# qurAI-amsterdam/SuperResolution_aniso_MRI

Hardware: AMD Instinct MI355X
Metric: training slices/sec (ae_combined, 160x160, latent=128) (higher is better)
Workload: dtype f32; 1 GPU; ACDC synthetic 12x(3x1x160x160) triplets, ae_combined latent=128 depth=32 scales=2, MSE synthesis loss (BASELINE configs[1]); global_batch_triplets=12, parallelism=dp1, init=reference Initializer, seed 892372, random weights, launch=captured HIP graph replay

## Files before the change

### superresolution_aniso_mri_amd/_hip.py

```python
import ctypes
import os
from ctypes import c_char_p, c_double, c_float, c_int, c_int64, c_size_t, c_void_p

import torch

_HERE = os.path.dirname(os.path.abspath(__file__))
LIB_PATH = os.path.join(_HERE, "libaesr_hip.so")
if os.environ.get("AESR_LIB"):
    import sys as _sys
    LIB_PATH = os.path.abspath(os.environ["AESR_LIB"])
    _sys.stderr.write("[aesr] AESR_LIB: loading the VARIANT library %s (not the shipped libaesr_hip.so)\n" % LIB_PATH)

P = c_void_p
IP = ctypes.POINTER(c_int)
FP = ctypes.POINTER(c_float)
DP = ctypes.POINTER(c_double)

class TripletDesc(ctypes.Structure):
    _fields_ = [("vol_off", ctypes.c_longlong), ("H", c_int), ("W", c_int), ("z_from", c_int), ("z_to", c_int), ("z_between", c_int),
                ("oy", c_int), ("ox", c_int), ("k", c_int), ("gain", c_float), ("cutoff", c_float)]


class WgradReduceJob(ctypes.Structure):
    _fields_ = [("workspace", c_void_p), ("dw", c_void_p), ("db", c_void_p), ("N", c_int), ("H", c_int), ("W", c_int), ("Cin", c_int),
# ... 110 lines not shown
    "aesr_conv2d_wino_fwd": (c_int, [P, P, P, P] + [c_int] * 6 + [c_float, P]),
    "aesr_conv2d_wino_dgrad": (c_int, [P, P, P, P] + [c_int] * 6 + [c_float, P]),
    "aesr_conv2d_wino_workspace_floats": (c_size_t, [c_int] * 6),
    "aesr_conv2d_wino_fwd_bn_supported": (c_int, [c_int] * 5),
    "aesr_conv2d_wino_fwd_bn": (c_int, [P, P, P, P, P, P] + [c_int] * 6 + [c_float, c_int, P]),
    "aesr_conv2d_wino_fwd_ws": (c_int, [P, P, P, P, P, c_size_t] + [c_int] * 6 + [c_float, P]),
    "aesr_conv2d_wino_dgrad_ws": (c_int, [P, P, P, P, P, c_size_t] + [c_int] * 6 + [c_float, P]),
    "aesr_conv2d_wino_fwd_up2": (c_int, [P, P, P, P] + [c_int] * 6 + [c_float, P]),
    "aesr_conv2d_wino_dgrad_sum2": (c_int, [P, P, P] + [c_int] * 5 + [P]),
    "aesr_conv2d_wgrad_up2_supported": (c_int, [c_int, c_int]),
    "aesr_conv2d_wgrad_up2": (c_int, [P, P, P, P, P] + [c_int] * 5 + [P]),
    "aesr_conv2d_wgrad_partial": (c_int, [P, P, P] + [c_int] * 8 + [P]),
    "aesr_conv2d_wgrad_reduce_many": (c_int, [ctypes.POINTER(WgradReduceJob), c_int, P]),
    "aesr_comm_rccl_version": (c_int, [IP]),
    "aesr_comm_unique_id": (c_int, [c_char_p]),
    "aesr_comm_init": (c_int, [c_char_p, c_int, c_int, ctypes.POINTER(c_void_p)]),
    "aesr_comm_destroy": (c_int, [P]),
    "aesr_comm_abort": (c_int, [P]),
    "aesr_comm_allreduce": (c_int, [P, P, c_size_t, c_int, c_int, P]),
    "aesr_comm_allreduce_many": (c_int, [P, ctypes.POINTER(c_void_p), ctypes.POINTER(c_size_t), c_int, c_int, c_int, P]),
    "aesr_comm_broadcast": (c_int, [P, P, c_size_t, c_int, c_int, P]),
}
SIGNATURES_PREPROC = {
    "aesr_inplane_out_size": (c_int, [c_int, c_double]),
    "aesr_inplane_workspace_bytes": (c_size_t, [c_int, c_int]),
    "aesr_inplane_resample": (c_int, [P, P, P] + [c_int] * 5 + [DP, c_int, DP, c_int, IP, DP, IP, DP, c_int, P]),
}
SIGNATURES_DATAPREP = {
    "aesr_thick_slices_out_slices": (c_int, [c_int, c_int]),
    "aesr_thick_slices_store_bytes": (c_int, [c_int, P, P]),
    "aesr_thick_slices": (c_int, [P, P, c_int, c_int, c_int, c_int, DP, c_int, P]),
    "aesr_triplet_assemble_raw": (c_int, [P, ctypes.POINTER(TripletDesc), c_int, c_int, P, P, P]),
}
P2P_HANDLE_BYTES, P2P_SLOTS = 64, 32
COMM_ID_BYTES = 128
COMM_F32, COMM_F64, COMM_SUM, COMM_MAX = 0, 1, 0, 1

ACT_NONE, ACT_LRELU, ACT_RELU, ACT_SIGMOID = 0, 1, 2, 3
BN_NONE, BN_POOL, BN_UP = 0, 1, 2
RS_POOL, RS_NEAREST, RS_BILINEAR = 1, 2, 3
BN_NWG = 512
REDUCE_MAX_JOBS = 16
MSE_NPART = 512
MSE3_WS = 3 * 256 + 1
LPIPS_NCH = 64


def _load():
    if not os.path.exists(LIB_PATH):
        raise RuntimeError(
            "libaesr_hip.so not found at %s -- build it with `python __graft_entry__.py` (or `make -C "
            "superresolution_aniso_mri_amd/csrc`). The HIP extension is mandatory: there is no CPU/eager fallback." % LIB_PATH)
    lib = ctypes.CDLL(LIB_PATH)
    for name, (res, args) in list(SIGNATURES.items()) + list(SIGNATURES_PREPROC.items()) + list(SIGNATURES_DATAPREP.items()):
        fn = getattr(lib, name, None)
        if fn is None:
            raise RuntimeError("libaesr_hip.so does not export %s (stale build?)" % name)
        fn.restype, fn.argtypes = res, args
    return lib


lib = _load()


def last_error():
    return lib.aesr_last_error_string().decode("utf-8", "replace")


def check(rc, what):
    if rc != 0:
        raise RuntimeError("%s failed (code %d): %s" % (what, rc, last_error()))


def check_device_watchdogs(where):
    nb = int(lib.aesr_bn_fused1_timeouts())
    if nb:
        raise RuntimeError("%s: the one-launch BatchNorm kernel's grid barrier gave up %d time(s) in this process -- its workgroups were not all "
                           "resident (the device is shared with another grid-barrier kernel: set AESR_BN_FUSED=0); results since are not "
                           "trustworthy; nothing was written" % (where, nb))
    n = int(lib.aesr_conv2d_wino_ring_timeouts())
    if n:
        raise RuntimeError("%s: the ring convolution kernel's arrival-counter watchdog fired %d time(s) in this process -- activations / "
                           "gradients computed since are not trustworthy (csrc/conv_wino_ring.hip: wait_full); nothing was written" % (where, n))


def ptr(t):
    if t is None:
# ... 35 lines not shown
```

### superresolution_aniso_mri_amd/csrc/aesr_api.hip

```cpp
#include <stdarg.h>
#include <stdio.h>
#include <stdlib.h>
#include <string.h>

#include <map>
#include <mutex>
#include <tuple>

#include "../../include/aesr_hip.h"
#include "../../include/aesr_hip_dataprep.h"
#include "aesr_kernels.h"

static thread_local char g_err[512] = "";
void aesr_set_error(const char* fmt, ...) {
    va_list ap;
    va_start(ap, fmt);
    vsnprintf(g_err, sizeof(g_err), fmt, ap);
    va_end(ap);
}

static void cout_padding(int Cout, int* CoutP, int* NB) {
    if (Cout <= 16) { *CoutP = 16; *NB = 1; }
    else if (Cout <= 32) { *CoutP = 32; *NB = 2; }
    else { *CoutP = round_up(Cout, 64); *NB = 4; }
}

static bool conv_dims_ok(int N, int H, int W, int Cin, int Cout) {
    if (N < 1 || H < 1 || W < 1 || Cin < 1 || Cout < 1) return false;
    if (N > (1 << 24) || H > (1 << 15) || W > (1 << 15) || Cin > (1 << 15) || Cout > (1 << 15)) return false;
    const unsigned long long px = (unsigned long long)N * (unsigned)(H + 2) * (unsigned)(W + 2);
    return px * (unsigned long long)(Cin > Cout ? Cin : Cout) < 0x1C000000ull;
}
#define AESR_CHECK_DIMS(who, N, H, W, Cin, Cout)                                                                                            \
    do {                                                                                                                                    \
        if (!conv_dims_ok(N, H, W, Cin, Cout)) {                                                                                            \
            aesr_set_error("%s: %d x %d x %d with %d -> %d channels is empty or beyond the kernels' 32-bit element offsets (469M elements)", who, N, H, \
                           W, Cin, Cout);                                                                                                   \
            return AESR_ERR_UNSUPPORTED;                                                                                                    \
        }                                                                                                                                   \
    } while (0)

struct ConvPlan { int TI, TH, TW, NB, MBW, CinP, CoutP, NT, ksplit; };
static std::mutex g_plan_mu;
// ... 717 lines not shown
    a.TH = H < 16 ? H : 16; a.TW = W < 16 ? W : 16;
    while ((size_t)(a.TH + 2) * (a.TW + 2) * (Cin + 1) * 4 > 60 * 1024 && a.TH > 1) a.TH /= 2;
    a.tiles_y = ceil_div(H, a.TH); a.tiles_x = ceil_div(W, a.TW); a.ntiles = N * a.tiles_y * a.tiles_x;
    int nwg = a.ntiles < SMALL_WGRAD_NWG ? a.ntiles : SMALL_WGRAD_NWG;
    if (int e = aesr_launch_cout1_wgrad(a, nwg, (hipStream_t)stream)) return e;
    return aesr_launch_sum_partials(workspace, nwg, Cin * 9 + 1, dw, Cin * 9, db, (hipStream_t)stream);
}

int aesr_conv2d_cout1_dgrad(const float* dy, const float* w, const float* y_saved, float* dx, float* workspace, int N, int H,
                            int W, int Cin, int mask_act, float slope, void* stream) {
    AESR_CHECK_ARG(dy && w && dx && workspace && N > 0 && H > 0 && W > 0, "aesr_conv2d_cout1_dgrad: null pointer or empty shape");
    AESR_CHECK_ARG(thin_channels_ok(Cin), "aesr_conv2d_cout1_dgrad: Cin=%d must be 4 times a power of two (4..256)", Cin);
    if (int e = aesr_launch_thin_cout1_flip(w, workspace, Cin, (hipStream_t)stream)) return e;
    ThinArgs a;
    memset(&a, 0, sizeof(a));
    a.s = dy; a.w = workspace; a.ysave = y_saved; a.out = dx;
    a.N = N; a.Hs = H; a.Ws = W; a.Ho = H; a.Wo = W; a.C = Cin; a.ps = 0;
    a.act = ACT_NONE; a.mask_act = y_saved ? mask_act : ACT_NONE; a.slope = slope;
    return aesr_launch_thin_expand(a, (hipStream_t)stream);
}

int aesr_conv2d_cout1_dgrad_pre(const float* dy, const float* w_flipped, const float* y_saved, float* dx, int N, int H, int W, int Cin,
                                int mask_act, float slope, void* stream) {
    AESR_CHECK_ARG(dy && w_flipped && dx && N > 0 && H > 0 && W > 0, "aesr_conv2d_cout1_dgrad_pre: null pointer or empty shape");
    AESR_CHECK_ARG(thin_channels_ok(Cin), "aesr_conv2d_cout1_dgrad_pre: Cin=%d must be 4 times a power of two (4..256)", Cin);
    ThinArgs a;
    memset(&a, 0, sizeof(a));
    a.s = dy; a.w = w_flipped; a.ysave = y_saved; a.out = dx;
    a.N = N; a.Hs = H; a.Ws = W; a.Ho = H; a.Wo = W; a.C = Cin; a.ps = 0;
    a.act = ACT_NONE; a.mask_act = y_saved ? mask_act : ACT_NONE; a.slope = slope;
    return aesr_launch_thin_expand(a, (hipStream_t)stream);
}

size_t aesr_stemconv_folded_floats(int C1) { return (size_t)2 * 9 * C1; }

int aesr_stemconv_fold(const float* w_stem, const float* b_stem, const float* w1, float* folded, int Cs, int C1, void* stream) {
    AESR_CHECK_ARG(w_stem && w1 && folded && Cs > 0 && C1 > 0, "aesr_stemconv_fold: bad arguments");
    return aesr_launch_thin_stem_fold(w_stem, b_stem, w1, folded, Cs, C1, (hipStream_t)stream);
}

int aesr_stemconv_fwd(const float* x, const float* folded, const float* b1, float* out, int N, int H, int W, int C1,
                      int stem_pad, int act, float slope, void* stream) {
    AESR_CHECK_ARG(x && folded && out && N > 0 && H > 0 && W > 0 && stem_pad >= 0, "aesr_stemconv_fwd: bad arguments");
    AESR_CHECK_ARG(thin_channels_ok(C1), "aesr_stemconv_fwd: C1=%d must be 4 times a power of two (4..256)", C1);
    ThinArgs a;
    memset(&a, 0, sizeof(a));
    a.s = x; a.w = folded; a.be = folded + (size_t)9 * C1; a.b = b1; a.out = out;
    a.N = N; a.Hs = H; a.Ws = W; a.Ho = H + 2 * stem_pad; a.Wo = W + 2 * stem_pad; a.C = C1; a.ps = stem_pad;
    a.act = act; a.mask_act = ACT_NONE; a.slope = slope;
    return aesr_launch_thin_expand(a, (hipStream_t)stream);
}

size_t aesr_stemconv_workspace_floats(int C1) { return (size_t)(THIN_NWG + 1) * 19 * C1; }

int aesr_stemconv_wgrad(const float* x, const float* g, const float* w_stem, const float* b_stem, const float* w1,
                        float* dw_stem, float* db_stem, float* dw1, float* db1, float* workspace, int N, int H, int W, int Cs,
                        int C1, int stem_pad, void* stream) {
    AESR_CHECK_ARG(x && g && w_stem && w1 && dw_stem && dw1 && workspace, "aesr_stemconv_wgrad: null pointer");
    AESR_CHECK_ARG(N > 0 && H > 0 && W > 0 && Cs > 0 && stem_pad >= 0, "aesr_stemconv_wgrad: bad shape");
    AESR_CHECK_ARG(thin_channels_ok(C1), "aesr_stemconv_wgrad: C1=%d must be 4 times a power of two (4..256)", C1);
    AESR_CHECK_ARG(!db_stem || b_stem, "aesr_stemconv_wgrad: db_stem needs b_stem");
    ThinArgs a;
    memset(&a, 0, sizeof(a));
    a.s = x; a.t = g; a.partial = workspace;
    a.N = N; a.Hs = H; a.Ws = W; a.Ho = H + 2 * stem_pad; a.Wo = W + 2 * stem_pad; a.C = C1; a.ps = stem_pad; a.with_be = 1;
    float* R = workspace + (size_t)THIN_NWG * 19 * C1;
// ... 452 lines not shown
```

### superresolution_aniso_mri_amd/csrc/aesr_kernels.h

```cpp
#pragma once
#include "aesr_common.h"

struct IgemmArgs {
    const float* in; const float* wpk; const float* bias; const float* ysave; float* out;
    int N, H, W, Cin, CinP, Cout, CoutP, Ho, Wo, pad;
    int TI, TH, TW, tiles_y, tiles_x, nitems, dbg;
    int NT;
    int ksplit;
    float* dbgbuf;
    int act, mask_act;
    float slope;
};
int aesr_launch_conv_igemm(const IgemmArgs& a, int KS, int NB, int MBW, hipStream_t st);
int aesr_launch_conv_ksplit_fixup(const float* partial, const float* bias, const float* ysave, float* out, size_t nelem, int Cout,
                                  int ksplit, int act, int mask_act, float slope, hipStream_t st);
int aesr_launch_pack_weights(const float* w, float* p, int Cout, int Cin, int KS, int KinP, int NoutP, int TN, int transpose, hipStream_t st);

struct WinoArgs {
    const float* in; const float* upk; const float* bias; const float* ysave; float* out;
    int N, H, W, Cin, CinP, Cout, CoutP;
    int TI, THt, TWt;
    int regs_y, regs_x, nitems;
    unsigned m_ncot, m_regs_x, m_regs_y;
    int act, mask_act;
// ... 71 lines not shown
    const float* in; const float* dout; float* partial;
    int N, H, W, Cin, Cout, Ho, Wo, pad;
};
struct Cout1WgradArgs {
    const float* x; const float* dy; float* partial;
    int N, H, W, Cin, TH, TW, tiles_y, tiles_x, ntiles;
};
struct Cout1FwdArgs {
    const float* x; const float* w; const float* bias; float* out;
    int N, H, W, Cin, TH, TW, tiles_y, tiles_x, act;
    float slope;
};
int aesr_launch_cout1_fwd(const Cout1FwdArgs& a, hipStream_t st);
int aesr_launch_smallcin_fwd(const SmallArgs& a, hipStream_t st);
int aesr_launch_smallcin_dgrad(const SmallDgradArgs& a, hipStream_t st);
int aesr_launch_sum_partials(const float* partial, int np, int n, float* out0, int n0, float* out1, hipStream_t st);
int aesr_launch_smallcin_wgrad(const SmallWgradArgs& a, int nwg, hipStream_t st);
int aesr_launch_cout1_wgrad(const Cout1WgradArgs& a, int nwg, hipStream_t st);

struct ThinArgs {
    const float* s;
    const float* w;
    const float* be;
    const float* b;
    const float* ysave;
    float* out;
    const float* t;
    float* partial;
    int N, Hs, Ws, Ho, Wo, C, ps;
    int act, mask_act;
    float slope;
    int with_be;
    int tiles_y, tiles_x, ntiles;
};
int aesr_launch_thin_expand(ThinArgs a, hipStream_t st);
int aesr_launch_thin_reduce(ThinArgs a, int nwg, hipStream_t st);
int aesr_launch_thin_collapse(const float* x, const float* w, const float* bias, float* out, int N, int H, int W, int C, int act,
                              float slope, hipStream_t st);
int aesr_launch_thin_stem_fold(const float* ws, const float* bs, const float* w1, float* folded, int Cs, int C1, hipStream_t st);
int aesr_launch_thin_stem_finish(const float* R, const float* ws, const float* bs, const float* w1, float* dws, float* dbs,
                                 float* dw1, float* db1, int Cs, int C1, hipStream_t st);
int aesr_launch_thin_cout1_flip(const float* w, float* wexp, int Cin, hipStream_t st);
int aesr_launch_thin_cout1_finish(const float* R, float* dw, float* db, int Cin, hipStream_t st);

struct BnGroups { int G; int nstart[5]; };
struct BnApplyArgs {
    const float* y; const float* scale; const float* shift; float* out;
    int N, H, W, C, Ho, Wo, mode;
    BnGroups gr;
};
struct BnBwdArgs {
    const float* gout; const float* y; const float* mean; const float* invstd; const float* scale; const float* coef;
    float* partial; float* dpre;
    int N, H, W, C, Ho, Wo, mode, act;
    float slope;
    BnGroups gr;
    unsigned long long m_hw, m_w;
    int k_hw, k_w;
};
struct BnFusedArgs;
struct BnP2P { int world, rank, slot; const unsigned* gen; void* peers[8]; };
int aesr_launch_p2p_tick(unsigned* gen, hipStream_t st);
bool aesr_bn_fused1_ok(int N, int H, int W, int C, int pool, int G, int backward);
unsigned aesr_bn_fused_timeouts_impl();
int aesr_bn_fused_run(const float* y, const float* gout, float* out, float* rec, unsigned* bar, const float* gamma, const float* beta,
                      float* running_mean, float* running_var, long long* nbt, float* mean, float* invstd, float* scale, float* shift, float* coef,
                      float* dgamma, float* dbeta, int N, int H, int W, int C, int pool, int G, const int* nstart, const double* counts,
                      float momentum, float eps, int update_running, int act, float slope, int backward, const BnP2P* p2p, hipStream_t st);
int aesr_launch_bn_stats(const float* y, float* partial, int HW, int C, const BnGroups& gr, int nwg, hipStream_t st);
int aesr_launch_bn_reduce(const float* partial, double* sums, int nwg, int C, int G, hipStream_t st);
int aesr_launch_bn_finalize(const double* sums, const double* counts, const float* gamma, const float* beta, float* rm, float* rv,
                            long long* nbt, float* mean, float* invstd, float* scale, float* shift, int C, int G, float momentum,
                            float eps, int train, int update_running, hipStream_t st);
int aesr_launch_bn_reduce_finalize(const float* partial, int nwg, const double* counts, const float* gamma, const float* beta,
                                   float* running_mean, float* running_var, long long* nbt, float* mean, float* invstd,
                                   float* scale, float* shift, int C, int G, float momentum, float eps, int update_running,
// ... 60 lines not shown
```

### superresolution_aniso_mri_amd/csrc/conv_thin.hip

```cpp
#include "aesr_kernels.h"
#include "aesr_pack_dev.h"

#define THIN_TH 8
#ifndef THIN_ETH
#define THIN_ETH 16
#endif
#define THIN_XS 68

__host__ __device__ __forceinline__ int thin_tw(int C4) { return 256 / C4 < 64 ? 256 / C4 : 64; }

template <int TH = THIN_TH>
__device__ __forceinline__ void thin_stage(const ThinArgs& a, float (*xs)[THIN_XS], int n, int y0, int x0, int TW) {
    const int PW = TW + 2;
    for (int q = threadIdx.x; q < (TH + 2) * PW; q += 256) {
        const int r = q / PW, c = q - r * PW;
        const int sy = y0 + r - 1 - a.ps, sx = x0 + c - 1 - a.ps;
        float v = 0.f;
        if (sy >= 0 && sy < a.Hs && sx >= 0 && sx < a.Ws) v = a.s[((size_t)n * a.Hs + sy) * a.Ws + sx];
        xs[r][c] = v;
    }
}

__global__ __launch_bounds__(256) void thin_expand_kernel(ThinArgs a) {
    __shared__ float xs[THIN_ETH + 2][THIN_XS];
    const int C4 = a.C >> 2, TW = thin_tw(C4);
    const int tid = threadIdx.x, c4 = tid % C4, pl = tid / C4;
    int tile = blockIdx.x;
    const int tx = tile % a.tiles_x;
    tile /= a.tiles_x;
    const int ty = tile % a.tiles_y;
    const int n = tile / a.tiles_y;
    const int y0 = ty * THIN_ETH, x0 = tx * TW;
    thin_stage<THIN_ETH>(a, xs, n, y0, x0, TW);
    f32x4 w[9];
#pragma unroll
    for (int t = 0; t < 9; ++t) w[t] = *(const f32x4*)(a.w + t * a.C + c4 * 4);
    const f32x4 b0 = a.b ? *(const f32x4*)(a.b + c4 * 4) : (f32x4){0.f, 0.f, 0.f, 0.f};
    f32x4 bfull = b0;
    if (a.be) {
#pragma unroll
        for (int t = 0; t < 9; ++t) bfull += *(const f32x4*)(a.be + t * a.C + c4 * 4);
    }
    __syncthreads();
    const int ox = x0 + pl;
    if (pl >= TW || ox >= a.Wo) return;
    const bool xedge = a.be && (ox == 0 || ox == a.Wo - 1);
    const bool sigm = a.act == ACT_SIGMOID;
    const float nslope = a.act == ACT_LRELU ? a.slope : (a.act == ACT_RELU ? 0.f : 1.f);
    const bool fastact = !sigm && nslope >= 0.f && nslope <= 1.f;
#pragma unroll 4
    for (int r = 0; r < THIN_ETH; ++r) {
        const int oy = y0 + r;
        if (oy >= a.Ho) break;
        f32x4 acc = bfull;
        if (xedge || (a.be && (oy == 0 || oy == a.Ho - 1))) {
            acc = b0;
            for (int t = 0; t < 9; ++t) {
                const int yy = oy + t / 3 - 1, xx = ox + t % 3 - 1;
                if (yy >= 0 && yy < a.Ho && xx >= 0 && xx < a.Wo) acc += *(const f32x4*)(a.be + t * a.C + c4 * 4);
            }
        }
#pragma unroll
        for (int t = 0; t < 9; ++t) {
            const float v = xs[r + t / 3][pl + t % 3];
#pragma unroll
            for (int e = 0; e < 4; ++e) acc[e] = fmaf(w[t][e], v, acc[e]);
        }
        const size_t o = (((size_t)n * a.Ho + oy) * a.Wo + ox) * a.C + c4 * 4;
        if (fastact) {
#pragma unroll
            for (int e = 0; e < 4; ++e) acc[e] = fmaxf(acc[e], acc[e] * nslope);
        } else {
#pragma unroll
            for (int e = 0; e < 4; ++e) acc[e] = act_apply(acc[e], a.act, a.slope);
        }
        if (a.ysave) {
            const f32x4 ys = *(const f32x4*)(a.ysave + o);
#pragma unroll
            for (int e = 0; e < 4; ++e) acc[e] *= act_grad_from_output(ys[e], a.mask_act, a.slope);
        }
        *(f32x4*)(a.out + o) = acc;
    }
}

template <bool WITH_BE>
__global__ __launch_bounds__(256) void thin_reduce_kernel(ThinArgs a) {
    __shared__ float xs[THIN_TH + 2][THIN_XS];
    extern __shared__ __attribute__((aligned(16))) float red[];
    constexpr int NROW = WITH_BE ? 19 : 10;
    const int C4 = a.C >> 2, TW = thin_tw(C4);
    const int tid = threadIdx.x, c4 = tid % C4, pl = tid / C4;
    const int lane = tid & 63, wave = tid >> 6;
    f32x4 accW[9], accB[9];
    float accs = 0.f;
#pragma unroll
    for (int t = 0; t < 9; ++t) {
        accW[t] = (f32x4){0.f, 0.f, 0.f, 0.f};
        accB[t] = (f32x4){0.f, 0.f, 0.f, 0.f};
    }
    const int tpi = a.tiles_y * a.tiles_x;
    for (int tile = blockIdx.x; tile < a.ntiles; tile += gridDim.x) {
        const int n = tile / tpi;
        const int trem = tile - n * tpi;
        const int ty = trem / a.tiles_x, tx = trem - ty * a.tiles_x;
        const int y0 = ty * THIN_TH, x0 = tx * TW;
        __syncthreads();
        thin_stage(a, xs, n, y0, x0, TW);
        const int ox = x0 + pl;
        const bool xin = pl < TW && ox < a.Wo;
        const int plr = pl < TW ? pl : 0;
        f32x4 g[THIN_TH];
#pragma unroll
        for (int r = 0; r < THIN_TH; ++r) {
            const int oy = y0 + r;
            g[r] = (f32x4){0.f, 0.f, 0.f, 0.f};
            if (xin && oy < a.Ho) g[r] = *(const f32x4*)(a.t + (((size_t)n * a.Ho + oy) * a.Wo + ox) * a.C + c4 * 4);
        }
        float mxf[3];
        mxf[0] = (ox - 1 >= 0) ? 1.f : 0.f;
        mxf[1] = 1.f;
        mxf[2] = (ox + 1 < a.Wo) ? 1.f : 0.f;
        __syncthreads();
#pragma unroll
        for (int r = 0; r < THIN_TH; ++r) {
            const int oy = y0 + r;
#pragma unroll
            for (int t = 0; t < 9; ++t) {
                const float v = xs[r + t / 3][plr + t % 3];
#pragma unroll
                for (int e = 0; e < 4; ++e) accW[t][e] = fmaf(g[r][e], v, accW[t][e]);
            }
            if (WITH_BE) {
#pragma unroll
                for (int dy = 0; dy < 3; ++dy) {
                    const int yy = oy + dy - 1;
                    const float myf = (yy >= 0 && yy < a.Ho) ? 1.f : 0.f;
#pragma unroll
                    for (int dx = 0; dx < 3; ++dx) {
                        const float m = myf * mxf[dx];
#pragma unroll
                        for (int e = 0; e < 4; ++e) accB[dy * 3 + dx][e] = fmaf(g[r][e], m, accB[dy * 3 + dx][e]);
                    }
                }
            }
            if (c4 == 0 && xin && oy < a.Ho) accs += xs[r + 1][plr + 1];
        }
    }
    for (int m = C4; m < 64; m <<= 1) {
#pragma unroll
        for (int t = 0; t < 9; ++t)
#pragma unroll
            for (int e = 0; e < 4; ++e) {
                accW[t][e] += __shfl_xor(accW[t][e], m, 64);
                if (WITH_BE) accB[t][e] += __shfl_xor(accB[t][e], m, 64);
            }
    }
    for (int m = 1; m < 64; m <<= 1) accs += __shfl_xor(accs, m, 64);
    __syncthreads();
    if (lane < C4) {
        float* rw = red + (size_t)wave * NROW * a.C;
#pragma unroll
        for (int t = 0; t < 9; ++t) {
            *(f32x4*)(rw + t * a.C + c4 * 4) = accW[t];
// ... 102 lines not shown
            sb += wv * (double)R[(9 + t) * C1 + co];
        }
        redw[threadIdx.x] = sw;
        redb[threadIdx.x] = sb;
        __syncthreads();
        for (int h = 128; h > 0; h >>= 1) {
            if ((int)threadIdx.x < h) {
                redw[threadIdx.x] += redw[threadIdx.x + h];
                redb[threadIdx.x] += redb[threadIdx.x + h];
            }
            __syncthreads();
        }
        if (threadIdx.x == 0) {
            dws[c] = (float)redw[0];
            if (dbs) dbs[c] = (float)redb[0];
        }
        return;
    }
    const int tid = (blockIdx.x - Cs) * 256 + threadIdx.x, nth = (gridDim.x - Cs) * 256;
    for (int o = tid; o < C1 * Cs * 9; o += nth) {
        const int t = o % 9, c = (o / 9) % Cs, co = o / (9 * Cs);
        float v = R[t * C1 + co] * ws[c];
        if (bs) v = fmaf(R[(9 + t) * C1 + co], bs[c], v);
        dw1[o] = v;
    }
    if (db1)
        for (int co = tid; co < C1; co += nth) db1[co] = R[(9 + 4) * C1 + co];
}

__global__ __launch_bounds__(256) void thin_cout1_flip_kernel(const float* __restrict__ w, float* __restrict__ wexp, int Cin) {
    cout1_flip_elements(w, wexp, Cin, blockIdx.x * 256 + threadIdx.x, gridDim.x * 256);
}

__global__ __launch_bounds__(256) void thin_cout1_finish_kernel(const float* __restrict__ R, float* __restrict__ dw,
                                                                float* __restrict__ db, int Cin) {
    for (int o = blockIdx.x * 256 + threadIdx.x; o < 9 * Cin; o += gridDim.x * 256) {
        const int ci = o / 9, k = o - ci * 9;
        dw[o] = R[(8 - k) * Cin + ci];
    }
    if (db && blockIdx.x == 0 && threadIdx.x == 0) db[0] = R[9 * Cin];
}


static bool thin_shape_ok(const ThinArgs& a) {
    const int C4 = a.C / 4;
    return a.C >= 4 && a.C % 4 == 0 && a.C <= 256 && (C4 & (C4 - 1)) == 0;
}

int aesr_launch_thin_expand(ThinArgs a, hipStream_t st) {
    if (!thin_shape_ok(a)) {
        aesr_set_error("thin conv: C=%d must be 4 times a power of two (4..256)", a.C);
        return AESR_ERR_ARG;
    }
    const int TW = thin_tw(a.C / 4);
    a.tiles_y = ceil_div(a.Ho, THIN_ETH);
    a.tiles_x = ceil_div(a.Wo, TW);
    a.ntiles = a.N * a.tiles_y * a.tiles_x;
    hipLaunchKernelGGL(thin_expand_kernel, dim3(a.ntiles), dim3(256), 0, st, a);
    AESR_LAUNCH_CHECK("thin_expand");
    return AESR_OK;
}

int aesr_launch_thin_reduce(ThinArgs a, int nwg, hipStream_t st) {
    if (!thin_shape_ok(a)) {
        aesr_set_error("thin conv: C=%d must be 4 times a power of two (4..256)", a.C);
        return AESR_ERR_ARG;
    }
    const int TW = thin_tw(a.C / 4);
    a.tiles_y = ceil_div(a.Ho, THIN_TH);
    a.tiles_x = ceil_div(a.Wo, TW);
    a.ntiles = a.N * a.tiles_y * a.tiles_x;
    const int nrow = a.with_be ? 19 : 10;
    const size_t shmem = (size_t)4 * nrow * a.C * sizeof(float);
    if (a.with_be)
        hipLaunchKernelGGL(thin_reduce_kernel<true>, dim3(nwg), dim3(256), shmem, st, a);
    else
        hipLaunchKernelGGL(thin_reduce_kernel<false>, dim3(nwg), dim3(256), shmem, st, a);
    AESR_LAUNCH_CHECK("thin_reduce");
    return AESR_OK;
}

int aesr_launch_thin_collapse(const float* x, const float* w, const float* bias, float* out, int N, int H, int W, int C, int act,
                              float slope, hipStream_t st) {
    const int C4 = C / 4;
    if (C < 4 || C % 4 != 0 || C > 256 || (C4 & (C4 - 1)) != 0) {
        aesr_set_error("thin conv: C=%d must be 4 times a power of two (4..256)", C);
        return AESR_ERR_ARG;
    }
    const int TW = thin_tw(C4), TH = H < 20 ? H : 20;
    const int tiles_y = ceil_div(H, TH), tiles_x = ceil_div(W, TW - 2);
    hipLaunchKernelGGL(thin_collapse_kernel, dim3(N * tiles_y * tiles_x), dim3(256), 0, st, x, w, bias, out, N, H, W, C, TH, tiles_y,
                       tiles_x, act, slope);
    AESR_LAUNCH_CHECK("thin_collapse");
    return AESR_OK;
}

int aesr_launch_thin_stem_fold(const float* ws, const float* bs, const float* w1, float* folded, int Cs, int C1, hipStream_t st) {
    hipLaunchKernelGGL(thin_stem_fold_kernel, dim3(ceil_div(9 * C1, 256)), dim3(256), 0, st, ws, bs, w1, folded, Cs, C1);
    AESR_LAUNCH_CHECK("thin_stem_fold");
    return AESR_OK;
}

int aesr_launch_thin_stem_finish(const float* R, const float* ws, const float* bs, const float* w1, float* dws, float* dbs,
                                 float* dw1, float* db1, int Cs, int C1, hipStream_t st) {
    int grid = ceil_div(C1 * Cs * 9, 256);
    if (grid > 64) grid = 64;
    hipLaunchKernelGGL(thin_stem_finish_kernel, dim3(Cs + grid), dim3(256), 0, st, R, ws, bs, w1, dws, dbs, dw1, db1, Cs, C1);
    AESR_LAUNCH_CHECK("thin_stem_finish");
    return AESR_OK;
}

int aesr_launch_thin_cout1_flip(const float* w, float* wexp, int Cin, hipStream_t st) {
    hipLaunchKernelGGL(thin_cout1_flip_kernel, dim3(ceil_div(9 * Cin, 256)), dim3(256), 0, st, w, wexp, Cin);
    AESR_LAUNCH_CHECK("thin_cout1_flip");
    return AESR_OK;
}

int aesr_launch_thin_cout1_finish(const float* R, float* dw, float* db, int Cin, hipStream_t st) {
    hipLaunchKernelGGL(thin_cout1_finish_kernel, dim3(ceil_div(9 * Cin, 256)), dim3(256), 0, st, R, dw, db, Cin);
    AESR_LAUNCH_CHECK("thin_cout1_finish");
    return AESR_OK;
}
```

### superresolution_aniso_mri_amd/engine.py

```python
import os
from ctypes import c_float

import torch
import torch.nn as nn

from . import _hip
from ._hip import lib, ptr, stream, check

LRELU_SLOPE = 0.01


class KernelProfiler:

    def __init__(self):
        self.records = []

    def begin(self, kind, flops, nbytes=0.0):
        e0 = torch.cuda.Event(enable_timing=True)
        e1 = torch.cuda.Event(enable_timing=True)
        e0.record(torch.cuda.current_stream())
        self.records.append((kind, flops, nbytes, e0, e1))

    def end(self):
        self.records[-1][4].record(torch.cuda.current_stream())

    def summary(self):
        torch.cuda.synchronize()
        out = {}
        for kind, flops, nbytes, e0, e1 in self.records:
            d = out.setdefault(kind, {"launches": 0, "flops": 0.0, "bytes": 0.0, "ms": 0.0})
            d["launches"] += 1
            d["flops"] += flops
            d["bytes"] += nbytes
            d["ms"] += e0.elapsed_time(e1)
        return out


PROFILER = None
TRACE = None
FUSE_STEM = os.environ.get("AESR_FUSE_STEM", "1") != "0"
USE_WINO = os.environ.get("AESR_WINO", "1") != "0"
FOLD_UPSAMPLE = os.environ.get("AESR_FOLD_UPSAMPLE", "1") != "0"
FUSE_EVAL_BN = os.environ.get("AESR_FUSE_EVAL_BN", "1") != "0"


def bn_fused_enabled():
    return os.environ.get("AESR_BN_FUSED", "1") != "0"


def bn_fused_pays(N, H, W, C):
    if N > int(os.environ.get("AESR_BN_FUSED_MAX_IMAGES", "9")):
        return False
    return float(N) * H * W * C * 4.0 <= float(os.environ.get("AESR_BN_FUSED_MAX_MB", "1000")) * 1e6


def wino_ok(cin, cout, ks, pad, transpose):
    return bool(USE_WINO and lib.aesr_conv2d_wino_supported(int(cin), int(cout), int(ks), int(pad), int(transpose)))


def wino_kind(n, h, w, cin, cout, transpose):
    k = lib.aesr_conv2d_wino_kernel(int(n), int(h), int(w), int(cin), int(cout), 3, 1, int(transpose))
    return {2: "conv_wino_res_f32", 3: "conv_wino_ring_f32"}.get(k, "conv_wino_f32")


def wino_workspace(like, n, h, w, cin, cout, transpose):
    nws = lib.aesr_conv2d_wino_workspace_floats(n, h, w, cin, cout, transpose)
    return (torch.empty((nws,), device=like.device, dtype=torch.float32), nws) if nws else (None, 0)


def wgrad_kind(cin, cout, ks, pad):
    return "conv_wgrad_wino_f32" if (ks == 3 and pad == 1 and lib.aesr_conv2d_wgrad_up2_supported(int(cin), int(cout))) else "conv_wgrad_f32"


# ... 513 lines not shown
        if _DEFERRED is not None:
            _DEFERRED.extend(j for j in reduce_jobs if j[4])
            flush_wgrad_reductions([j for j in reduce_jobs if not j[4]])
        else:
            flush_wgrad_reductions(reduce_jobs)
        return g, grads

    def _backward_steps(self, steps, saved, g, ngrad, need_input_grad, grads, G, ns, reduce_jobs):
        for k in range(len(steps) - 1, -1, -1):
            s = steps[k]
            if s.kind == "stemconv":
                if need_input_grad:
                    raise RuntimeError("the stem-folded pass has no input gradient (run the pass with fused=False)")
                xin = saved[k][0]
                _, H, W, _ = xin.shape
                dws, dbs = self._grad_dst(s.stem.weight, grads), self._grad_dst(s.stem.bias, grads)
                dw1 = self._grad_dst(s.mod.weight, grads)
                db1 = self._grad_dst(s.mod.bias, grads) if s.mod.bias is not None else None
                ws = _empty((lib.aesr_stemconv_workspace_floats(s.cout),), g)
                _pb("thin_reduce", 0.0, 4.0 * (ngrad * H * W + g.numel()))
                check(lib.aesr_stemconv_wgrad(ptr(xin), ptr(g), ptr(s.stem.weight), ptr(s.stem.bias), ptr(s.mod.weight),
                                              ptr(dws), ptr(dbs), ptr(dw1), ptr(db1), ptr(ws), ngrad, H, W, s.cs, s.cout,
                                              s.stem_pad, stream()), "aesr_stemconv_wgrad")
                _pe()
                g = None
                break
            if s.kind == "conv":
                xin, yout = saved[k][0], saved[k][1]
                N, H, W, _ = xin.shape
                N = ngrad
                if s.in_up2:
                    H, W = 2 * H, 2 * W
                Ho, Wo = (H, W) if s.s2d else s.out_hw(H, W)
                if k == len(steps) - 1 and s.act != _hip.ACT_NONE:
                    dpre = torch.empty_like(g)
                    check(lib.aesr_act_bwd(ptr(g), ptr(yout), ptr(dpre), g.numel(), s.act, s.slope, stream()), "aesr_act_bwd")
                    g = dpre
                dw_final = self._grad_dst(s.mod.weight, grads)
                dw = torch.empty((s.cout, s.cin, 1, 1), device=g.device) if s.s2d else dw_final
                db = self._grad_dst(s.mod.bias, grads) if s.mod.bias is not None else None
                if s.cin % 4 == 0 and s.cout % 4 == 0:
                    nws = lib.aesr_conv2d_wgrad_workspace_floats(N, H, W, s.cin, s.cout, s.ks, s.pad)
                    ws = _empty((nws,), g)
                    if s.s2d:
                        _pb(("wgrad", s.cin, s.cout, s.ks, s.pad), 2.0 * N * Ho * Wo * s.cout * s.ks * s.ks * s.cin)
                        check(lib.aesr_conv2d_wgrad(ptr(xin), ptr(g), ptr(dw), ptr(db), ptr(ws), N, H, W, s.cin, s.cout, s.ks,
                                                    s.pad, stream()), "aesr_conv2d_wgrad")
                        _pe()
                    else:
                        _pb(("wgrad", s.cin, s.cout, s.ks, s.pad), 2.0 * N * Ho * Wo * s.cout * s.ks * s.ks * s.cin)
                        check(lib.aesr_conv2d_wgrad_partial(ptr(xin), ptr(g), ptr(ws), N, H, W, s.cin, s.cout, s.ks, s.pad,
                                                            int(s.in_up2), stream()), "aesr_conv2d_wgrad_partial")
                        _pe()
                        direct = grads[s.mod.weight] is None and (db is None or grads[s.mod.bias] is None)
                        reduce_jobs.append((_hip.WgradReduceJob(ws.data_ptr(), dw.data_ptr(), db.data_ptr() if db is not None else None,
                                                                N, H, W, s.cin, s.cout, s.ks, s.pad), ws, dw, db, direct))
                elif s.cin <= 4 and s.ks == 1 and db is not None:
                    ws = _empty((lib.aesr_small_wgrad_workspace_floats(s.cout * (s.cin + 1)),), g)
                    check(lib.aesr_conv2d_smallcin_wgrad(ptr(xin), ptr(g), ptr(dw), ptr(db), ptr(ws), N, H, W, s.cin, s.cout,
                                                         s.pad, stream()), "aesr_conv2d_smallcin_wgrad")
                elif s.cout == 1 and s.ks == 3 and s.pad == 1 and db is not None:
                    ws = _empty((lib.aesr_conv2d_cout1_workspace_floats(s.cin),), g)
                    _pb("thin_reduce", 0.0, 4.0 * (N * H * W * s.cin + g.numel()))
                    check(lib.aesr_conv2d_cout1_wgrad(ptr(xin), ptr(g), ptr(dw), ptr(db), ptr(ws), N, H, W, s.cin, stream()),
                          "aesr_conv2d_cout1_wgrad")
                    _pe()
# ... 226 lines not shown
```

Baseline: 15930 slices/s.

## Fuse Cout=1 final conv backward: act-grad, wgrad, dgrad in one pass

Adds a fused backward kernel for the last 3x3 conv with one output channel. A single thin reduce pass applies the activation gradient on the fly, accumulates weight and bias partials, and computes the input gradient with the previous layer's activation mask applied. A small kernel then sums the partials in double precision. This replaces the separate act_bwd, wgrad reduce and dgrad expand launches and their extra reads of the activations. The cost is higher register pressure in the reduce kernel.

```diff
diff --git a/include/aesr_hip_train.h b/include/aesr_hip_train.h
--- /dev/null
+++ b/include/aesr_hip_train.h
@@ -0,0 +1,24 @@
+#ifndef AESR_HIP_TRAIN_H
+#define AESR_HIP_TRAIN_H
+
+#include <stddef.h>
+
+#include "aesr_hip.h"
+
+#ifdef __cplusplus
+extern "C" {
+#endif
+
+size_t aesr_conv2d_cout1_bwd_workspace_floats(int Cin);
+
+int aesr_conv2d_cout1_bwd(const float* x,
+                          const float* dout,
+                          const float* out,
+                          const float* w_flipped,
+                          float* dw, float* db, float* dx, float* workspace, int N, int H, int W, int Cin, int act, float slope,
+                          int mask_act, float mask_slope, void* stream);
+
+#ifdef __cplusplus
+}
+#endif
+#endif
diff --git a/superresolution_aniso_mri_amd/_hip.py b/superresolution_aniso_mri_amd/_hip.py
--- a/superresolution_aniso_mri_amd/_hip.py
+++ b/superresolution_aniso_mri_amd/_hip.py
@@ -166,6 +166,10 @@
     "aesr_thick_slices": (c_int, [P, P, c_int, c_int, c_int, c_int, DP, c_int, P]),
     "aesr_triplet_assemble_raw": (c_int, [P, ctypes.POINTER(TripletDesc), c_int, c_int, P, P, P]),
 }
+SIGNATURES_TRAIN = {
+    "aesr_conv2d_cout1_bwd_workspace_floats": (c_size_t, [c_int]),
+    "aesr_conv2d_cout1_bwd": (c_int, [P] * 8 + [c_int] * 5 + [c_float, c_int, c_float, P]),
+}
 P2P_HANDLE_BYTES, P2P_SLOTS = 64, 32
 COMM_ID_BYTES = 128
 COMM_F32, COMM_F64, COMM_SUM, COMM_MAX = 0, 1, 0, 1
@@ -186,7 +190,8 @@
             "libaesr_hip.so not found at %s -- build it with `python __graft_entry__.py` (or `make -C "
             "superresolution_aniso_mri_amd/csrc`). The HIP extension is mandatory: there is no CPU/eager fallback." % LIB_PATH)
     lib = ctypes.CDLL(LIB_PATH)
-    for name, (res, args) in list(SIGNATURES.items()) + list(SIGNATURES_PREPROC.items()) + list(SIGNATURES_DATAPREP.items()):
+    for name, (res, args) in (list(SIGNATURES.items()) + list(SIGNATURES_PREPROC.items()) + list(SIGNATURES_DATAPREP.items())
+                                   + list(SIGNATURES_TRAIN.items())):
         fn = getattr(lib, name, None)
         if fn is None:
             raise RuntimeError("libaesr_hip.so does not export %s (stale build?)" % name)
diff --git a/superresolution_aniso_mri_amd/csrc/aesr_api.hip b/superresolution_aniso_mri_amd/csrc/aesr_api.hip
--- a/superresolution_aniso_mri_amd/csrc/aesr_api.hip
+++ b/superresolution_aniso_mri_amd/csrc/aesr_api.hip
@@ -9,6 +9,7 @@
 
 #include "../../include/aesr_hip.h"
 #include "../../include/aesr_hip_dataprep.h"
+#include "../../include/aesr_hip_train.h"
 #include "aesr_kernels.h"
 
 static thread_local char g_err[512] = "";
@@ -792,6 +793,26 @@
     return aesr_launch_thin_expand(a, (hipStream_t)stream);
 }
 
+size_t aesr_conv2d_cout1_bwd_workspace_floats(int Cin) { return Cin > 0 ? (size_t)(THIN_NWG + 1) * 10 * Cin : 0; }
+
+int aesr_conv2d_cout1_bwd(const float* x, const float* dout, const float* out, const float* w_flipped, float* dw, float* db, float* dx,
+                          float* workspace, int N, int H, int W, int Cin, int act, float slope, int mask_act, float mask_slope,
+                          void* stream) {
+    AESR_CHECK_ARG(x && dout && w_flipped && dw && db && dx && workspace, "aesr_conv2d_cout1_bwd: null pointer");
+    AESR_CHECK_ARG(N > 0 && H > 0 && W > 0, "aesr_conv2d_cout1_bwd: empty shape");
+    AESR_CHECK_ARG(thin_channels_ok(Cin), "aesr_conv2d_cout1_bwd: Cin=%d must be 4 times a power of two (4..256)", Cin);
+    AESR_CHECK_ARG(act >= ACT_NONE && act <= ACT_SIGMOID && mask_act >= ACT_NONE && mask_act <= ACT_SIGMOID,
+                   "aesr_conv2d_cout1_bwd: unknown activation (act=%d, mask_act=%d)", act, mask_act);
+    AESR_CHECK_ARG(out || act == ACT_NONE, "aesr_conv2d_cout1_bwd: out (the saved output) is needed for act=%d", act);
+    ThinArgs a;
+    memset(&a, 0, sizeof(a));
+    a.s = dout; a.sout = act == ACT_NONE ? nullptr : out; a.t = x; a.partial = workspace; a.w = w_flipped; a.out = dx;
+    a.N = N; a.Hs = H; a.Ws = W; a.Ho = H; a.Wo = W; a.C = Cin; a.ps = 0; a.with_be = 0;
+    a.act = act; a.slope = slope; a.mask_act = mask_act; a.mask_slope = mask_slope;
+    if (int e = aesr_launch_thin_reduce_dx(a, THIN_NWG, (hipStream_t)stream)) return e;
+    return aesr_launch_thin_cout1_finish_sum(workspace, THIN_NWG, dw, db, Cin, (hipStream_t)stream);
+}
+
 size_t aesr_stemconv_folded_floats(int C1) { return (size_t)2 * 9 * C1; }
 
 int aesr_stemconv_fold(const float* w_stem, const float* b_stem, const float* w1, float* folded, int Cs, int C1, void* stream) {
diff --git a/superresolution_aniso_mri_amd/csrc/aesr_kernels.h b/superresolution_aniso_mri_amd/csrc/aesr_kernels.h
--- a/superresolution_aniso_mri_amd/csrc/aesr_kernels.h
+++ b/superresolution_aniso_mri_amd/csrc/aesr_kernels.h
@@ -127,9 +127,12 @@
     float slope;
     int with_be;
     int tiles_y, tiles_x, ntiles;
+    const float* sout;
+    float mask_slope;
 };
 int aesr_launch_thin_expand(ThinArgs a, hipStream_t st);
 int aesr_launch_thin_reduce(ThinArgs a, int nwg, hipStream_t st);
+int aesr_launch_thin_reduce_dx(ThinArgs a, int nwg, hipStream_t st);
 int aesr_launch_thin_collapse(const float* x, const float* w, const float* bias, float* out, int N, int H, int W, int C, int act,
                               float slope, hipStream_t st);
 int aesr_launch_thin_stem_fold(const float* ws, const float* bs, const float* w1, float* folded, int Cs, int C1, hipStream_t st);
@@ -137,6 +140,7 @@
                                  float* dw1, float* db1, int Cs, int C1, hipStream_t st);
 int aesr_launch_thin_cout1_flip(const float* w, float* wexp, int Cin, hipStream_t st);
 int aesr_launch_thin_cout1_finish(const float* R, float* dw, float* db, int Cin, hipStream_t st);
+int aesr_launch_thin_cout1_finish_sum(const float* partial, int np, float* dw, float* db, int Cin, hipStream_t st);
 
 struct BnGroups { int G; int nstart[5]; };
 struct BnApplyArgs {
diff --git a/superresolution_aniso_mri_amd/csrc/conv_thin.hip b/superresolution_aniso_mri_amd/csrc/conv_thin.hip
--- a/superresolution_aniso_mri_amd/csrc/conv_thin.hip
+++ b/superresolution_aniso_mri_amd/csrc/conv_thin.hip
@@ -18,6 +18,34 @@
         float v = 0.f;
         if (sy >= 0 && sy < a.Hs && sx >= 0 && sx < a.Ws) v = a.s[((size_t)n * a.Hs + sy) * a.Ws + sx];
         xs[r][c] = v;
+    }
+}
+
+#define THIN_NPV (((THIN_TH + 2) * 66 + 255) / 256)
+__device__ __forceinline__ void thin_stage_act(const ThinArgs& a, float (*xs)[THIN_XS], int n, int y0, int x0, int TW) {
+    const int PW = TW + 2;
+    const float* so = a.sout ? a.sout : a.s;
+    float pv[THIN_NPV], po[THIN_NPV];
+    bool in[THIN_NPV];
+#pragma unroll
+    for (int j = 0; j < THIN_NPV; ++j) {
+        const int q = threadIdx.x + j * 256;
+        const int r = q / PW, c = q - r * PW;
+        const int sy = y0 + r - 1 - a.ps, sx = x0 + c - 1 - a.ps;
+        in[j] = q < (THIN_TH + 2) * PW && sy >= 0 && sy < a.Hs && sx >= 0 && sx < a.Ws;
+        const size_t i = in[j] ? ((size_t)n * a.Hs + sy) * a.Ws + sx : 0;
+        pv[j] = a.s[i];
+        po[j] = so[i];
+    }
+#pragma unroll
+    for (int j = 0; j < THIN_NPV; ++j) {
+        const int q = threadIdx.x + j * 256;
+        const int r = q / PW, c = q - r * PW;
+        if (q < (THIN_TH + 2) * PW) {
+            float v = in[j] ? pv[j] : 0.f;
+            if (in[j] && a.sout) v = v * act_grad_from_output(po[j], a.act, a.slope);
+            xs[r][c] = v;
+        }
     }
 }
 
@@ -83,7 +111,7 @@
     }
 }
 
-template <bool WITH_BE>
+template <bool WITH_BE, bool WITH_DX = false>
 __global__ __launch_bounds__(256) void thin_reduce_kernel(ThinArgs a) {
     __shared__ float xs[THIN_TH + 2][THIN_XS];
     extern __shared__ __attribute__((aligned(16))) float red[];
@@ -98,6 +126,13 @@
         accW[t] = (f32x4){0.f, 0.f, 0.f, 0.f};
         accB[t] = (f32x4){0.f, 0.f, 0.f, 0.f};
     }
+    f32x4 w[WITH_DX ? 9 : 1];
+    if constexpr (WITH_DX) {
+#pragma unroll
+        for (int t = 0; t < 9; ++t) w[t] = *(const f32x4*)(a.w + t * a.C + c4 * 4);
+    }
+    const bool msig = WITH_DX && a.mask_act == ACT_SIGMOID;
+    const float mneg = (WITH_DX && a.mask_act == ACT_LRELU) ? a.mask_slope : 0.f;
     const int tpi = a.tiles_y * a.tiles_x;
     for (int tile = blockIdx.x; tile < a.ntiles; tile += gridDim.x) {
         const int n = tile / tpi;
@@ -105,7 +140,7 @@
         const int ty = trem / a.tiles_x, tx = trem - ty * a.tiles_x;
         const int y0 = ty * THIN_TH, x0 = tx * TW;
         __syncthreads();
-        thin_stage(a, xs, n, y0, x0, TW);
+        if constexpr (!WITH_DX) thin_stage(a, xs, n, y0, x0, TW);
         const int ox = x0 + pl;
         const bool xin = pl < TW && ox < a.Wo;
         const int plr = pl < TW ? pl : 0;
@@ -116,6 +151,7 @@
             g[r] = (f32x4){0.f, 0.f, 0.f, 0.f};
             if (xin && oy < a.Ho) g[r] = *(const f32x4*)(a.t + (((size_t)n * a.Ho + oy) * a.Wo + ox) * a.C + c4 * 4);
         }
+        if constexpr (WITH_DX) thin_stage_act(a, xs, n, y0, x0, TW);
         float mxf[3];
         mxf[0] = (ox - 1 >= 0) ? 1.f : 0.f;
         mxf[1] = 1.f;
@@ -124,11 +160,26 @@
 #pragma unroll
         for (int r = 0; r < THIN_TH; ++r) {
             const int oy = y0 + r;
+            f32x4 dx = {0.f, 0.f, 0.f, 0.f};
 #pragma unroll
             for (int t = 0; t < 9; ++t) {
                 const float v = xs[r + t / 3][plr + t % 3];
 #pragma unroll
                 for (int e = 0; e < 4; ++e) accW[t][e] = fmaf(g[r][e], v, accW[t][e]);
+                if constexpr (WITH_DX) {
+#pragma unroll
+                    for (int e = 0; e < 4; ++e) dx[e] = fmaf(w[t][e], v, dx[e]);
+                }
+            }
+            if constexpr (WITH_DX) {
+                if (msig) {
+#pragma unroll
+                    for (int e = 0; e < 4; ++e) dx[e] *= g[r][e] * (1.f - g[r][e]);
+                } else if (a.mask_act != ACT_NONE) {
+#pragma unroll
+                    for (int e = 0; e < 4; ++e) dx[e] *= g[r][e] > 0.f ? 1.f : mneg;
+                }
+                if (xin && oy < a.Ho) *(f32x4*)(a.out + (((size_t)n * a.Ho + oy) * a.Wo + ox) * a.C + c4 * 4) = dx;
             }
             if (WITH_BE) {
 #pragma unroll
@@ -297,6 +348,42 @@
     cout1_flip_elements(w, wexp, Cin, blockIdx.x * 256 + threadIdx.x, gridDim.x * 256);
 }
 
+__global__ __launch_bounds__(1024) void thin_cout1_finish_kernel(const float* __restrict__ partial, int np, float* __restrict__ dw,
+                                                                 float* __restrict__ db, int Cin) {
+    __shared__ double red[16][64];
+    const int n = 10 * Cin, nuse = 9 * Cin + 1;
+    const int col = threadIdx.x & 63, rl = threadIdx.x >> 6;
+    const int o = blockIdx.x * 64 + col;
+    double s = 0.0;
+    if (o < nuse) {
+        double s0 = 0.0, s1 = 0.0, s2 = 0.0, s3 = 0.0;
+        int p = rl;
+        for (; p + 48 < np; p += 64) {
+            const float v0 = partial[(size_t)p * n + o], v1 = partial[(size_t)(p + 16) * n + o];
+            const float v2 = partial[(size_t)(p + 32) * n + o], v3 = partial[(size_t)(p + 48) * n + o];
+            s0 += (double)v0;
+            s1 += (double)v1;
+            s2 += (double)v2;
+            s3 += (double)v3;
+        }
+        for (; p < np; p += 16) s0 += (double)partial[(size_t)p * n + o];
+        s = (s0 + s1) + (s2 + s3);
+    }
+    red[rl][col] = s;
+    __syncthreads();
+    if (rl == 0 && o < nuse) {
+        s = 0.0;
+#pragma unroll
+        for (int k = 0; k < 16; ++k) s += red[k][col];
+        if (o < 9 * Cin) {
+            const int t = o / Cin, ci = o - t * Cin;
+            dw[ci * 9 + 8 - t] = (float)s;
+        } else {
+            db[0] = (float)s;
+        }
+    }
+}
+
 __global__ __launch_bounds__(256) void thin_cout1_finish_kernel(const float* __restrict__ R, float* __restrict__ dw,
                                                                 float* __restrict__ db, int Cin) {
     for (int o = blockIdx.x * 256 + threadIdx.x; o < 9 * Cin; o += gridDim.x * 256) {
@@ -345,6 +432,21 @@
     return AESR_OK;
 }
 
+int aesr_launch_thin_reduce_dx(ThinArgs a, int nwg, hipStream_t st) {
+    if (!thin_shape_ok(a)) {
+        aesr_set_error("thin conv: C=%d must be 4 times a power of two (4..256)", a.C);
+        return AESR_ERR_ARG;
+    }
+    const int TW = thin_tw(a.C / 4);
+    a.tiles_y = ceil_div(a.Ho, THIN_TH);
+    a.tiles_x = ceil_div(a.Wo, TW);
+    a.ntiles = a.N * a.tiles_y * a.tiles_x;
+    const size_t shmem = (size_t)4 * 10 * a.C * sizeof(float);
+    hipLaunchKernelGGL((thin_reduce_kernel<false, true>), dim3(nwg), dim3(256), shmem, st, a);
+    AESR_LAUNCH_CHECK("thin_reduce_dx");
+    return AESR_OK;
+}
+
 int aesr_launch_thin_collapse(const float* x, const float* w, const float* bias, float* out, int N, int H, int W, int C, int act,
                               float slope, hipStream_t st) {
     const int C4 = C / 4;
@@ -386,3 +488,9 @@
     AESR_LAUNCH_CHECK("thin_cout1_finish");
     return AESR_OK;
 }
+
+int aesr_launch_thin_cout1_finish_sum(const float* partial, int np, float* dw, float* db, int Cin, hipStream_t st) {
+    hipLaunchKernelGGL(thin_cout1_finish_kernel, dim3(ceil_div(9 * Cin + 1, 64)), dim3(1024), 0, st, partial, np, dw, db, Cin);
+    AESR_LAUNCH_CHECK("thin_cout1_finish_sum");
+    return AESR_OK;
+}
diff --git a/superresolution_aniso_mri_amd/engine.py b/superresolution_aniso_mri_amd/engine.py
--- a/superresolution_aniso_mri_amd/engine.py
+++ b/superresolution_aniso_mri_amd/engine.py
@@ -39,6 +39,7 @@
 PROFILER = None
 TRACE = None
 FUSE_STEM = os.environ.get("AESR_FUSE_STEM", "1") != "0"
+FUSE_COUT1_BWD = os.environ.get("AESR_FUSE_COUT1_BWD", "1") != "0"
 USE_WINO = os.environ.get("AESR_WINO", "1") != "0"
 FOLD_UPSAMPLE = os.environ.get("AESR_FOLD_UPSAMPLE", "1") != "0"
 FUSE_EVAL_BN = os.environ.get("AESR_FUSE_EVAL_BN", "1") != "0"
@@ -618,6 +619,23 @@
                 if s.in_up2:
                     H, W = 2 * H, 2 * W
                 Ho, Wo = (H, W) if s.s2d else s.out_hw(H, W)
+                if (FUSE_COUT1_BWD and k == len(steps) - 1 and s.cout == 1 and s.ks == 3 and s.pad == 1 and _thin_channels(s.cin)
+                        and not s.s2d and not s.in_up2 and s.mod.bias is not None and (k > 0 or need_input_grad) and s.flipped is not None
+                        and s.packed_epoch == (self.weights_epoch, s.mod.weight._version, s.mod.weight.data_ptr())):
+                    mask_act, mslope = _hip.ACT_NONE, 0.0
+                    if k > 0 and steps[k - 1].kind in ("conv", "stemconv") and steps[k - 1].act != _hip.ACT_NONE:
+                        mask_act, mslope = steps[k - 1].act, steps[k - 1].slope
+                    if mask_act == _hip.ACT_NONE or saved[k - 1][1].data_ptr() == xin.data_ptr():
+                        dw, db = self._grad_dst(s.mod.weight, grads), self._grad_dst(s.mod.bias, grads)
+                        ws = _empty((lib.aesr_conv2d_cout1_bwd_workspace_floats(s.cin),), g)
+                        dx = _empty((N, H, W, s.cin), g)
+                        _pb("thin_reduce", 0.0, 4.0 * (2 * N * H * W * s.cin + 2 * N * H * W))
+                        check(lib.aesr_conv2d_cout1_bwd(ptr(xin), ptr(g), ptr(yout) if s.act != _hip.ACT_NONE else None, ptr(s.flipped), ptr(dw),
+                                                        ptr(db), ptr(dx), ptr(ws), N, H, W, s.cin, s.act, s.slope, mask_act, mslope, stream()),
+                              "aesr_conv2d_cout1_bwd")
+                        _pe()
+                        g = dx
+                        continue
                 if k == len(steps) - 1 and s.act != _hip.ACT_NONE:
                     dpre = torch.empty_like(g)
                     check(lib.aesr_act_bwd(ptr(g), ptr(yout), ptr(dpre), g.numel(), s.act, s.slope, stream()), "aesr_act_bwd")
```

After: 16110 slices/s, median of 6. 1.1% higher.
